# Lzcstan/DrugLAMP

Measured on AMD Instinct MI355X. Metric: drug-protein pairs/sec training step, higher is better.
Workload: dtype bf16; 1 GPU; DrugLAMP training step (cls step, epoch 1; fwd+bwd+grad all-reduce+AdamW), BindingDB-shaped synthetic pairs (512 drug nodes/tokens, 2304 protein tokens = 256 sites, pre-extracted 384-d/640-d LLM embeddings), global batch 256 = 256 per GPU x 1; per_gpu_batch=256, global_batch=256, parallelism=dp1, step_kind=cls, epoch=1, hip_graph=False, protein_seq_len=2304, distinct_batches=8, first_touch_steps=8, padding_rows=computed once, protein_cnn_rows=distinct rows, streams=independent branches on side HIP streams

## Files before the change

### druglamp_amd/_lib.py

```python
from __future__ import annotations

import ctypes as C
import os

import torch

_HERE = os.path.dirname(os.path.abspath(__file__))
_variant = os.environ.get("DL_USE_STUDY_LIB", "")
if _variant and not _variant.endswith(".so"):
    raise RuntimeError("DL_USE_STUDY_LIB=%s: the -DDL_STUDY build (libdruglamp_hip_study.so) was removed; commit 97fb613 is the last "
                       "that builds it (python -m druglamp_amd.build --study).  Only a variant library name (libdruglamp_hip_<variant>.so) "
                       "is accepted." % _variant)
LIB_PATH = os.path.join(_HERE, "lib", _variant or "libdruglamp_hip.so")

DL_F32, DL_BF16 = 0, 1

c_i64, c_i32, c_f32, c_u64, c_vp, c_sz = C.c_int64, C.c_int32, C.c_float, C.c_uint64, C.c_void_p, C.c_size_t


class ReduceItem(C.Structure):
    _fields_ = [
        ("kind", c_i32), ("out_dtype", c_i32),
        ("src", c_vp), ("out", c_vp),
        ("mn", c_i64), ("ldc", c_i64),
        ("N", c_i32), ("splits", c_i32), ("accumulate", c_i32), ("M", c_i32),
        ("cs_slabs", c_vp), ("cs_out", c_vp),
    ]


REDUCE_BATCH_MAX = 24
GEMM_GROUP_MAX = 16


class GemmArgs(C.Structure):
    _fields_ = [
        ("X", c_vp), ("ldx", c_i64), ("x_kslow", c_i32),
        ("W", c_vp), ("ldw", c_i64), ("w_kslow", c_i32),
        ("C", c_vp), ("ldc", c_i64),
        ("M", c_i64), ("N", c_i64), ("K", c_i64),
        ("in_dtype", c_i32), ("out_dtype", c_i32),
        ("bias", c_vp),
        ("residual", c_vp), ("ldr", c_i64),
        ("res_row_mod", c_i64),
        ("res_before_dropout", c_i32),
        ("act", c_i32),
        ("pre_out", c_vp), ("ldp", c_i64),
        ("dact_pre", c_vp), ("lddp", c_i64),
        ("dropout_p", c_f32), ("dropout_seed", c_u64),
        ("accumulate", c_i32),
        ("split_k", c_i32), ("workspace", c_vp), ("workspace_bytes", c_sz),
        ("x_colsum", c_vp),
        ("dropout_seed_offset", c_vp),
        ("algo", c_i32),
        ("tile_tickets", c_vp),
        ("deferred", C.POINTER(ReduceItem)),
        ("prof_tag", c_i32),
    ]


FLAG_PROT_PERIOD, FLAG_DRUG_TOKEN_PAD, FLAG_GCN_NODE_PAD, FLAG_PLAN_ROWS, FLAG_PAIR_INDEX = 1, 2, 4, 8, 16
FLAG_KEY_TABLE = 32
FLAG_MAP_COLS = 64
TAG_OTHER, TAG_QKV_OUT, TAG_FFN, TAG_CONV, TAG_WGRAD, TAG_ADAPTOR = 0, 1, 2, 3, 4, 5
TAG_NAMES = {0: "other", 1: "qkv_out", 2: "ffn", 3: "conv", 4: "wgrad", 5: "adaptor"}


class AttnFwdArgs(C.Structure):
    _fields_ = [
        ("Q", c_vp), ("K", c_vp), ("V", c_vp), ("O", c_vp), ("LSE", c_vp), ("raw_logits", c_vp),
        ("q_ps", c_i64), ("q_hs", c_i64), ("q_rs", c_i64),
        ("k_ps", c_i64), ("k_hs", c_i64), ("k_rs", c_i64),
        ("v_ps", c_i64), ("v_hs", c_i64), ("v_rs", c_i64),
        ("o_ps", c_i64), ("o_hs", c_i64), ("o_rs", c_i64), ("o_ss", c_i64),
        ("n_problems", c_i32), ("n_heads", c_i32), ("n_segments", c_i32), ("partner_shift", c_i32),
        ("Lq", c_i32), ("Lk", c_i32), ("head_dim", c_i32), ("dtype", c_i32),
        ("scale", c_f32),
        ("algo", c_i32),
        ("key_tail_rows", c_i32), ("key_tail_weight", c_f32),
    ]


class AttnBwdArgs(C.Structure):
    _fields_ = [
        ("Q", c_vp), ("K", c_vp), ("V", c_vp), ("O", c_vp), ("dO", c_vp),
        ("LSE", c_vp), ("Delta", c_vp),
        ("dQ", c_vp), ("dK", c_vp), ("dV", c_vp),
        ("q_ps", c_i64), ("q_hs", c_i64), ("q_rs", c_i64),
        ("k_ps", c_i64), ("k_hs", c_i64), ("k_rs", c_i64),
        ("v_ps", c_i64), ("v_hs", c_i64), ("v_rs", c_i64),
        ("o_ps", c_i64), ("o_hs", c_i64), ("o_rs", c_i64), ("o_ss", c_i64),
        ("do_ps", c_i64), ("do_hs", c_i64), ("do_rs", c_i64), ("do_ss", c_i64),
        ("dq_ps", c_i64), ("dq_hs", c_i64), ("dq_rs", c_i64),
        ("dk_ps", c_i64), ("dk_hs", c_i64), ("dk_rs", c_i64),
        ("dv_ps", c_i64), ("dv_hs", c_i64), ("dv_rs", c_i64),
        ("n_problems", c_i32), ("n_heads", c_i32), ("n_segments", c_i32), ("partner_shift", c_i32),
        ("Lq", c_i32), ("Lk", c_i32), ("head_dim", c_i32), ("dtype", c_i32),
        ("scale", c_f32),
        ("algo", c_i32),
        ("key_tail_rows", c_i32), ("key_tail_weight", c_f32),
    ]


class AttnProbsArgs(C.Structure):
    _fields_ = [
        ("Q", c_vp), ("K", c_vp), ("LSE", c_vp), ("out", c_vp), ("out_ld", c_i64),
        ("q_ps", c_i64), ("q_hs", c_i64), ("q_rs", c_i64),
        ("k_ps", c_i64), ("k_hs", c_i64), ("k_rs", c_i64),
        ("n_problems", c_i32), ("n_heads", c_i32), ("n_segments", c_i32), ("partner_shift", c_i32),
        ("Lq", c_i32), ("Lk", c_i32), ("head_dim", c_i32), ("dtype", c_i32),
        ("scale", c_f32),
        ("head_mean", c_i32), ("key_tail_rows", c_i32), ("key_tail_weight", c_f32), ("expand_tail", c_i32),
        ("workspace", c_vp), ("workspace_bytes", c_sz),
# ... 43 lines not shown
        ("Q", c_vp), ("K", c_vp), ("out", c_vp),
        ("q_index", c_vp), ("kv_index", c_vp), ("kv_row0", c_vp), ("kv_keys", c_vp), ("kv_tail_weight", c_vp), ("flags", c_vp),
        ("q_es", c_i64), ("q_rs", c_i64), ("k_rs", c_i64), ("out_ps", c_i64), ("out_rs", c_i64), ("kv_total_rows", c_i64),
        ("n_pairs", c_i32), ("n_q", c_i32), ("n_kv", c_i32), ("Lq", c_i32), ("head_dim", c_i32), ("dtype", c_i32),
        ("out_cols", c_i32), ("expand_tail", c_i32),
        ("scale", c_f32),
        ("key_tail_rows", c_i32),
    ]


class PgcaPairsProfileArgs(C.Structure):
    _fields_ = [
        ("Q", c_vp), ("K", c_vp), ("key_mass", c_vp), ("site_peak", c_vp), ("site_key", c_vp),
        ("q_index", c_vp), ("kv_index", c_vp), ("flags", c_vp),
        ("q_es", c_i64), ("q_rs", c_i64), ("k_es", c_i64), ("k_rs", c_i64), ("mass_ps", c_i64), ("site_ps", c_i64),
        ("n_pairs", c_i32), ("n_q", c_i32), ("n_kv", c_i32), ("Lq", c_i32), ("Lk", c_i32), ("head_dim", c_i32), ("dtype", c_i32),
        ("out_cols", c_i32),
        ("scale", c_f32),
        ("key_tail_rows", c_i32), ("key_tail_weight", c_f32),
        ("reserved", c_i32),
    ]


class PgcaPairsRaggedProfileArgs(C.Structure):
    _fields_ = [
        ("Q", c_vp), ("K", c_vp), ("key_mass", c_vp), ("site_peak", c_vp), ("site_key", c_vp),
        ("q_index", c_vp), ("kv_index", c_vp), ("kv_row0", c_vp), ("kv_keys", c_vp), ("kv_tail_weight", c_vp), ("flags", c_vp),
        ("q_es", c_i64), ("q_rs", c_i64), ("k_rs", c_i64), ("mass_ps", c_i64), ("site_ps", c_i64), ("kv_total_rows", c_i64),
        ("n_pairs", c_i32), ("n_q", c_i32), ("n_kv", c_i32), ("Lq", c_i32), ("head_dim", c_i32), ("dtype", c_i32),
        ("out_cols", c_i32),
        ("scale", c_f32),
        ("key_tail_rows", c_i32),
        ("reserved", c_i32),
    ]


class NtxentSide(C.Structure):
    _fields_ = [("q", c_vp), ("k", c_vp), ("n", c_i64), ("gid_offset", c_i64), ("lse", c_vp)]


class NtxentArgs(C.Structure):
    _fields_ = [("a", NtxentSide), ("b", NtxentSide), ("n_global", c_i64), ("d", c_i64), ("dtype", c_i32),
                ("temperature", c_f32)]


SIGNATURES = {
    "dl_last_error": (C.c_char_p, []),
    "dl_version": (c_i32, []),
    "dl_gemm_workspace_bytes": (c_sz, [C.POINTER(GemmArgs)]),
    "dl_gemm": (c_i32, [C.POINTER(GemmArgs), c_vp]),
    "dl_gemm_pair": (c_i32, [C.POINTER(GemmArgs), C.POINTER(GemmArgs), c_vp]),
    "dl_gemm_group_plan": (c_i32, [C.POINTER(GemmArgs), c_i32, C.POINTER(c_i32)]),
    "dl_gemm_group": (c_i32, [C.POINTER(GemmArgs), c_i32, c_vp]),
    "dl_reduce_batch": (c_i32, [C.POINTER(ReduceItem), c_i32, c_vp]),
    "dl_colsum": (c_i32, [c_vp, c_i64, c_i64, c_i64, c_i32, c_vp, c_i32, c_vp, c_sz, c_vp]),
    "dl_colsum_workspace_bytes": (c_sz, [c_i64, c_i64]),
    "dl_bn_workspace_bytes": (c_sz, [c_i64, c_i64]),
    "dl_bn_stats": (c_i32, [c_vp, c_i64, c_i64, c_i64, c_i64, c_i64, c_i32, c_vp, c_vp, c_sz, c_vp]),
    "dl_bn_apply_fwd": (c_i32, [c_vp, c_vp, c_vp, c_vp, c_vp, c_vp, c_i64, c_i64, c_i64, c_i64, c_i64, c_i32, c_vp]),
    "dl_bn_bwd_reduce": (c_i32, [c_vp, c_vp, c_vp, c_vp, c_i64, c_i64, c_i64, c_i64, c_i64, c_i32, c_vp, c_vp, c_sz, c_vp]),
    "dl_bn_tail_fix": (c_i32, [c_vp, c_vp, c_vp, c_vp, c_vp, c_vp, c_f32, c_i32, c_i64, c_i64, c_i64, c_i64, c_i32, c_vp]),
    "dl_bn_apply_relu_fwd": (c_i32, [c_vp, c_vp, c_vp, c_vp, c_vp, c_vp, c_i64, c_i64, c_i32, c_vp]),
    "dl_bn_relu_bwd": (c_i32, [c_vp, c_vp, c_vp, c_vp, c_vp, c_vp, c_f32, c_vp, c_vp, c_i64, c_i64, c_i32, c_vp, c_sz, c_vp]),
    "dl_bn_bwd_apply": (c_i32, [c_vp, c_vp, c_vp, c_vp, c_vp, c_vp, c_f32, c_i32, c_vp, c_i64, c_i64, c_i64, c_i64, c_i64,
                                c_i32, c_vp]),
    "dl_layernorm_fwd": (c_i32, [c_vp, c_i64, c_vp, c_vp, c_vp, c_i64, c_vp, c_vp, c_i64, c_i64, c_f32, c_i32, c_vp]),
    "dl_layernorm_bwd_workspace_bytes": (c_sz, [c_i64, c_i64]),
    "dl_layernorm_bwd": (c_i32, [c_vp, c_i64, c_i64, c_vp, c_i64, c_vp, c_vp, c_vp, c_vp, c_i64, c_vp, c_i64, c_vp, c_vp,
                                 c_i32, c_i64, c_i64, c_i32, c_vp, c_sz, C.POINTER(ReduceItem), c_vp]),
    "dl_attn_fwd": (c_i32, [C.POINTER(AttnFwdArgs), c_vp]),
    "dl_attn_bwd": (c_i32, [C.POINTER(AttnBwdArgs), c_vp]),
    "dl_attn_probs_workspace_bytes": (c_sz, [C.POINTER(AttnProbsArgs)]),
    "dl_attn_probs": (c_i32, [C.POINTER(AttnProbsArgs), c_vp]),
    "dl_pgca_pairs_fwd": (c_i32, [C.POINTER(PgcaPairsArgs), c_vp]),
    "dl_pgca_pairs_ragged_fwd": (c_i32, [C.POINTER(PgcaPairsRaggedArgs), c_vp]),
    "dl_pgca_pairs_probs": (c_i32, [C.POINTER(PgcaPairsProbsArgs), c_vp]),
    "dl_pgca_pairs_ragged_probs": (c_i32, [C.POINTER(PgcaPairsRaggedProbsArgs), c_vp]),
    "dl_pgca_pairs_profile": (c_i32, [C.POINTER(PgcaPairsProfileArgs), c_vp]),
    "dl_pgca_pairs_ragged_profile": (c_i32, [C.POINTER(PgcaPairsRaggedProfileArgs), c_vp]),
    "dl_token_gate_fwd": (c_i32, [c_vp, c_vp, c_vp, c_vp, c_i64, c_i64, c_i64, c_i32, c_i32, c_i32, c_vp]),
    "dl_token_gate_bwd": (c_i32, [c_vp, c_vp, c_vp, c_vp, c_vp, c_i64, c_i64, c_i64, c_i32, c_i32, c_i32, c_vp]),
    "dl_gate_dpre": (c_i32, [c_vp, c_vp, c_vp, c_vp, c_i64, c_i64, c_i32, c_i32, c_vp]),
    "dl_add_rowmod_dropout": (c_i32, [c_vp, c_vp, c_vp, c_i64, c_i64, c_i64, c_f32, c_u64, c_vp, c_i32, c_vp]),
    "dl_dropout_apply": (c_i32, [c_vp, c_vp, c_i64, c_i64, c_i64, c_i64, c_f32, c_u64, c_vp, c_i32, c_vp]),
    "dl_fill_pool": (c_i32, [c_vp, c_vp, c_vp, c_i64, c_i64, c_i64, c_i32, c_i32, c_i32, c_vp]),
    "dl_cnn_sitepool_fwd": (c_i32, [c_vp, c_vp, c_i64, c_i64, c_i64, c_i32, c_i32, c_i32, c_vp]),
    "dl_cnn_sitepool_bwd": (c_i32, [c_vp, c_vp, c_i64, c_i64, c_i64, c_i32, c_i32, c_i32, c_vp]),
    "dl_bn_stats_finalize": (c_i32, [c_vp, c_i64, c_i64, c_i64, c_i64, c_i64, c_vp, c_i32, c_i64, c_f32, c_f32, c_vp, c_vp, c_vp, c_vp, c_vp, c_vp, c_vp, c_sz, c_vp]),
    "dl_bn_finalize": (c_i32, [c_vp, c_i64, c_f32, c_f32, c_vp, c_vp, c_vp, c_vp, c_vp, c_i64, c_vp]),
    "dl_interleave_streams": (c_i32, [c_vp, c_vp, c_i64, c_i64, c_i32, c_i32, c_vp]),
    "dl_norm_adjacency": (c_i32, [c_vp, c_vp, c_i64, c_i32, c_i32, c_vp]),
    "dl_graph_aggregate": (c_i32, [c_vp, c_vp, c_vp, c_i64, c_i32, c_i32, c_i32, c_i32, c_i32, c_vp]),
    "dl_concat2": (c_i32, [c_vp, c_vp, c_vp, c_i64, c_i64, c_i64, c_i32, c_vp]),
    "dl_gather_pad": (c_i32, [c_vp, c_vp, c_vp, c_vp, c_i64, c_i64, c_i64, c_i32, c_i32, c_vp]),
    "dl_embed_pad": (c_i32, [c_vp, c_vp, c_vp, c_vp, c_i64, c_i64, c_i32, c_i32, c_i32, c_i32, c_vp]),
    "dl_weight_prep": (c_i32, [c_vp, c_vp, c_i32, c_i32, c_vp]),
    "dl_gelu_bwd": (c_i32, [c_vp, c_vp, c_vp, c_i64, c_i32, c_vp]),
    "dl_cast": (c_i32, [c_vp, c_i32, c_vp, c_i32, c_i64, c_vp]),
    "dl_rowmod_sum": (c_i32, [c_vp, c_vp, c_i64, c_i64, c_i64, c_i32, c_i32, c_vp]),
    "dl_cos_rowloss_fwd": (c_i32, [c_vp, c_vp, c_vp, c_vp, c_i64, c_i64, c_vp]),
    "dl_cos_rowloss_bwd": (c_i32, [c_vp, c_vp, c_f32, c_vp, c_i64, c_i64, c_vp]),
    "dl_ntxent_fwd_ex": (c_i32, [C.POINTER(NtxentArgs), c_vp, c_vp, c_vp, c_vp]),
    "dl_ntxent_bwd_ex": (c_i32, [C.POINTER(NtxentArgs), c_f32, c_vp, c_vp, c_vp]),
    "dl_ntxent_workspace_bytes": (c_sz, [c_i64, c_i64]),
    "dl_ntxent_fwd": (c_i32, [c_vp, c_vp, c_i64, c_i64, c_f32, c_vp, c_vp, c_vp, c_sz, c_vp]),
    "dl_ntxent_bwd": (c_i32, [c_vp, c_vp, c_i64, c_i64, c_f32, c_vp, c_f32, c_vp, c_vp, c_vp]),
# ... 118 lines not shown
```

### druglamp_amd/functional.py

```python
from __future__ import annotations

import functools
import contextlib
import os
import math
import weakref
from typing import List, Optional, Sequence

import torch

from . import ops

_param_epoch = 0
def _maybe_deferring():
    return contextlib.nullcontext() if os.environ.get("DL_DEFER_REDUCTIONS", "1") == "0" else ops.deferred_reductions()


def _deferring(fn):
    if os.environ.get("DL_DEFER_REDUCTIONS", "1") == "0":
        return fn

    @functools.wraps(fn)
    def wrapped(*a, **k):
        with ops.deferred_reductions():
# ... 519 lines not shown
    if not xp.is_contiguous():
        return ops.cast(x.contiguous(), dtype)
    inv = [0] * len(perm)
    for i, d in enumerate(perm):
        inv[d] = i
    return ops.cast(xp, dtype).permute(inv)


class CastFn(torch.autograd.Function):
    @staticmethod
    def forward(ctx, x, dtype):
        ctx.src = x.dtype
        return _cast_keep_layout(x, dtype)

    @staticmethod
    def backward(ctx, dy):
        return _cast_keep_layout(dy, ctx.src), None


def cast(x: torch.Tensor, dtype: torch.dtype) -> torch.Tensor:
    return x if x.dtype == dtype else CastFn.apply(x, dtype)


@torch.no_grad()
def attention_maps(x, blk, H: int, paired: bool):
    S, B, L, d = x.shape
    hd = d // H
    M = B * L
    maps = []
    qkvs = []
    for s in range(S):
        ps = blk.stream_params(s)
        xn, _, _ = ops.layernorm_fwd(x[s].reshape(M, d).contiguous(), ps[0].detach(), ps[1].detach(), 1e-6)
        w = lowp((ps[2], ps[4], ps[6]), x.dtype)
        b = lowp((ps[3], ps[5], ps[7]), torch.float32)
        qkvs.append(ops.gemm(xn, w, M=M, N=3 * d, K=d, bias=b))
    qs = (L * 3 * d, hd, 3 * d)

    def raw_of(qbuf, kbuf):
        raw = torch.empty((B, H, L, L), dtype=torch.float32, device=x.device)
        scratch = torch.empty((M, d), dtype=x.dtype, device=x.device)
        ops.attn_fwd(qbuf, kbuf[:, d:], kbuf[:, 2 * d:], n_problems=B, n_heads=H, n_segments=1, partner_shift=0, Lq=L,
                     Lk=L, head_dim=hd, scale=1.0 / math.sqrt(hd), q_strides=qs, k_strides=qs, v_strides=qs,
                     out=scratch, o_strides=(L * d, hd, d), o_ss=0, need_lse=False, raw_logits=raw)
        return torch.softmax(raw, dim=-1)

    w = raw_of(qkvs[0], qkvs[0])
    gw = raw_of(qkvs[1], qkvs[0]) if paired else None
    return w, gw


def _wgrad(g, x, M, N, K, ldx, ldw, want_bias=True, out_w=None, out_b=None):
    db = (out_b if out_b is not None else torch.empty(M, dtype=torch.float32, device=g.device)) if want_bias else None
    dw = ops.gemm(g, x, M=M, N=N, K=K, x_kslow=True, w_kslow=True, ldx=ldx, ldw=ldw, out_dtype=torch.float32,
                  split_k=0, x_colsum=db, out=out_w)
    return dw, db


class CosRowLossFn(torch.autograd.Function):

    @staticmethod
    def forward(ctx, x, y):
        x = x.float().contiguous()
        y = y.detach().float().contiguous()
        rows = ops.cos_rowloss_fwd(x, y)
        ctx.save_for_backward(x, y)
        return rows

    @staticmethod
    def backward(ctx, drows):
        x, y = ctx.saved_tensors
        dx = ops.cos_rowloss_bwd(x, y, 1.0)
        return dx * drows.unsqueeze(-1), None


class CrossEntropyRowsFn(torch.autograd.Function):

    @staticmethod
    def forward(ctx, logits, labels, C, ignore_index):
        logits = logits if logits.stride(-1) == 1 else logits.contiguous()
        labels = labels.reshape(-1).contiguous()
        out2, lse = ops.ce_rows_fwd(logits, labels, C, ignore_index)
        ctx.save_for_backward(logits, labels, lse, out2)
        ctx.cfg = (C, ignore_index)
        return out2[0]

    @staticmethod
    def backward(ctx, g):
        logits, labels, lse, out2 = ctx.saved_tensors
        C, ignore_index = ctx.cfg
        return ops.ce_rows_bwd(logits, labels, C, ignore_index, lse, out2, g.float().contiguous()), None, None, None


class NTXentFn(torch.autograd.Function):

    @staticmethod
    def forward(ctx, q, k, temperature, global_batch=False):
        import torch.distributed as dist
        if q.dtype not in (torch.float32, torch.bfloat16):
            q = q.float()
        q = q.contiguous()
        k = k.to(q.dtype).contiguous()
        world = dist.get_world_size() if (global_batch and dist.is_available() and dist.is_initialized()) else 1
        n = q.shape[0]
        if world > 1:
            rank = dist.get_rank()
# ... 267 lines not shown
        ctx.cfg = (x.shape, x.dtype)
        return x.mean(dim=1, dtype=torch.float32)

    @staticmethod
    def backward(ctx, g):
        (B, L, C), dt = ctx.cfg
        return (g * (1.0 / L)).to(dt).unsqueeze(1).expand(B, L, C)


class GraphAggregateFn(torch.autograd.Function):

    @staticmethod
    def _check(ahat, feat):
        if not (feat.is_cuda and feat.shape[-1] == 128 and ahat.dtype == feat.dtype and feat.dtype in (torch.float32, torch.bfloat16)):
            raise RuntimeError("GraphAggregateFn: device tensors of width 128 in one of fp32 / bf16 expected (got %s %s, %s %s): "
                               "there is no torch fallback" % (tuple(ahat.shape), ahat.dtype, tuple(feat.shape), feat.dtype))

    @staticmethod
    def forward(ctx, ahat, feat):
        GraphAggregateFn._check(ahat, feat)
        ctx.save_for_backward(ahat)
        return ops.graph_aggregate(ahat, feat, transpose=False)

    @staticmethod
    def backward(ctx, dout):
        (ahat,) = ctx.saved_tensors
        return None, ops.graph_aggregate(ahat, dout.contiguous(), transpose=True)


class EmbeddingFn(torch.autograd.Function):

    @staticmethod
    def forward(ctx, ids, weight, padding_idx):
        ctx.save_for_backward(ids)
        ctx.wshape = tuple(weight.shape)
        ctx.padding_idx = padding_idx
        return weight.detach()[ids]

    @staticmethod
    def backward(ctx, dy):
        (ids,) = ctx.saved_tensors
        V, D = ctx.wshape
        Vp, Dp = (V + 7) // 8 * 8, (D + 7) // 8 * 8
        flat = ids.reshape(-1)
        M = flat.numel()
        cdt = dy.dtype if dy.dtype in (torch.bfloat16, torch.float32) else torch.float32
        onehot = torch.zeros((M, Vp), dtype=cdt, device=dy.device)
        onehot.scatter_(1, flat.unsqueeze(1), 1.0)
        g = dy.reshape(M, D)
        if Dp != D or g.dtype != cdt or not g.is_contiguous():
            gp = torch.zeros((M, Dp), dtype=cdt, device=dy.device)
            gp[:, :D] = g
            g = gp
        dw = ops.gemm(onehot, g, M=Vp, N=Dp, K=M, x_kslow=True, w_kslow=True, ldx=Vp, ldw=Dp, out_dtype=torch.float32,
                      split_k=0)
        dw = dw[:V, :D]
        if ctx.padding_idx is not None:
            dw[ctx.padding_idx].zero_()
        return None, dw, None



class EmbedPadFn(torch.autograd.Function):

    @staticmethod
    def forward(ctx, ids, weight, fill, padding_idx):
        ctx.save_for_backward(ids)
        ctx.wshape = tuple(weight.shape)
        ctx.padding_idx = padding_idx
        return ops.embed_pad(ids, weight.detach(), fill, _CNN_HALO)

    @staticmethod
    def backward(ctx, dy):
        (ids,) = ctx.saved_tensors
        V, D = ctx.wshape
        B, LP, C = dy.shape
        Vp = (V + 7) // 8 * 8
        R = B * LP
        cdt = dy.dtype
        onehot = torch.zeros((B, LP, Vp), dtype=cdt, device=dy.device)
        onehot[:, _CNN_HALO:LP - _CNN_HALO].scatter_(2, ids.unsqueeze(-1), 1.0)
        g = dy.contiguous().reshape(R, C)
        dw = ops.gemm(onehot.reshape(R, Vp), g, M=Vp, N=C, K=R, x_kslow=True, w_kslow=True, ldx=Vp, ldw=C,
                      out_dtype=torch.float32, split_k=0)
        dw = dw[:V, :D]
        if ctx.padding_idx is not None:
            dw[ctx.padding_idx].zero_()
        return None, dw, None, None


class EmbedRowsFn(torch.autograd.Function):

    @staticmethod
    def forward(ctx, ids, weight, fill, padding_idx, src, period):
        ctx.save_for_backward(ids, src)
        ctx.wshape = tuple(weight.shape)
        ctx.padding_idx = padding_idx
        return ops.embed_rows(ids, weight.detach(), fill, src, period)

    @staticmethod
    def backward(ctx, dy):
        ids, src = ctx.saved_tensors
        V, D = ctx.wshape
        R, C = dy.shape
        Vp = (V + 7) // 8 * 8
        cdt = dy.dtype
        srcl = src.long()
        tok = ids.reshape(-1)[srcl.clamp(min=0)]
        onehot = torch.zeros((R, Vp), dtype=cdt, device=dy.device)
        onehot.scatter_(1, tok.unsqueeze(1), (srcl >= 0).to(cdt).unsqueeze(1))
        g = dy.contiguous()
        dw = ops.gemm(onehot, g, M=Vp, N=C, K=R, x_kslow=True, w_kslow=True, ldx=Vp, ldw=C, out_dtype=torch.float32, split_k=0)
        dw = dw[:V, :D]
        if ctx.padding_idx is not None:
            dw[ctx.padding_idx].zero_()
        return None, dw, None, None, None, None


class ExpandRowsFn(torch.autograd.Function):

    @staticmethod
    def forward(ctx, z, row_of, rep):
        ctx.save_for_backward(rep)
        return ops.rows_gather(z, row_of)

    @staticmethod
    def backward(ctx, dout):
        (rep,) = ctx.saved_tensors
        return ops.rows_sum_strided(dout.contiguous(), rep), None, None


class SitePoolRowsFn(torch.autograd.Function):

    @staticmethod
    def forward(ctx, z, row_of, rep, B, L, site_len):
        ctx.save_for_backward(row_of, rep)
        ctx.cfg = (L, site_len)
        return ops.cnn_sitepool_rows_fwd(z, row_of, B, L, site_len)

    @staticmethod
    def backward(ctx, dout):
        row_of, rep = ctx.saved_tensors
        L, site_len = ctx.cfg
        return ops.cnn_sitepool_rows_bwd(dout, rep, row_of, L, site_len), None, None, None, None, None


class SitePoolFn(torch.autograd.Function):

    @staticmethod
    def forward(ctx, z, site_len):
        B, L, C = z.shape
        ctx.cfg = (L, site_len)
        return ops.cnn_sitepool_fwd(z.contiguous(), L, 0, site_len)

    @staticmethod
    def backward(ctx, dout):
        L, site_len = ctx.cfg
        return ops.cnn_sitepool_bwd(dout, L, 0, site_len), None


class FillPoolFn(torch.autograd.Function):

    @staticmethod
    def forward(ctx, x, site_len, out_dtype):
        ctx.cfg = (tuple(x.shape), x.dtype, int(site_len))
# ... 198 lines not shown
```

### druglamp_amd/ops.py

```python
from __future__ import annotations

import contextlib
import ctypes as C
import math
import os
from typing import Optional

import torch

from . import _lib
from ._lib import (DL_BF16, DL_F32, AttnBwdArgs, AttnFwdArgs, AttnProbsArgs, GemmArgs, PgcaPairsArgs, PgcaPairsProbsArgs, PgcaPairsProfileArgs,
                   PgcaPairsRaggedArgs, PgcaPairsRaggedProbsArgs, PgcaPairsRaggedProfileArgs, check)

_DT = {torch.float32: DL_F32, torch.bfloat16: DL_BF16}


def _dt(t: torch.Tensor) -> int:
    try:
        return _DT[t.dtype]
    except KeyError:
        raise TypeError("druglamp_amd: unsupported dtype %s (float32 / bfloat16 only)" % t.dtype)


_raw_stream = getattr(torch._C, "_cuda_getCurrentRawStream", None)
# ... 77 lines not shown
    a.bias = _ptr(bias)
    a.residual = _ptr(residual)
    a.ldr = N if residual is None else residual.stride(-2)
    a.res_row_mod = res_row_mod
    a.res_before_dropout = int(res_before_dropout)
    a.act = act
    a.pre_out = _ptr(pre_out)
    a.ldp = N
    a.dact_pre = _ptr(dact_pre)
    a.lddp = N
    a.dropout_p = float(dropout_p)
    a.dropout_seed = int(seed)
    a.accumulate = int(accumulate)
    a.split_k = split_k
    a.x_colsum = _ptr(x_colsum)
    a.dropout_seed_offset = _seed_offset_ptr(x.device) if dropout_p > 0 else None
    a.algo = algo
    a.tile_tickets = _tickets_ptr(x.device)
    a.prof_tag = _lib.TAG_WGRAD if (x_kslow and w_kslow and _prof_tag != _lib.TAG_CONV) else _prof_tag
    return a, out


def gemm(x: torch.Tensor, w: torch.Tensor, **kw) -> torch.Tensor:
    a, out = _gemm_args(x, w, **kw)
    accumulate, x_colsum = kw.get("accumulate", False), kw.get("x_colsum")
    if (_wgroup is not None and a.x_kslow and a.w_kslow and a.split_k == 0 and not accumulate
            and (a.K <= group_wgrad_max_k or a.M * a.N < group_wgrad_small_mn)
            and x.dtype == torch.bfloat16 and out.dtype == torch.float32 and a.bias is None and a.residual is None and not a.act):
        _wgroup.append((a, out, x_colsum, x, w))
        return out
    _gemm_launch(a, out, x, accumulate, x_colsum)
    return out


def _gemm_launch(a, out, x, accumulate, x_colsum) -> None:
    L = _lib.lib()
    if accumulate and (_pending or _wgroup):
        flush_reductions()
    nbytes = L.dl_gemm_workspace_bytes(C.byref(a))
    item = None
    if nbytes:
        if _pending is not None and not accumulate:
            ws = torch.empty(nbytes, dtype=torch.uint8, device=x.device)
            item = _lib.ReduceItem()
            a.deferred = C.pointer(item)
        else:
            ws = _ws.get(nbytes, x.device)
        a.workspace, a.workspace_bytes = ws.data_ptr(), ws.numel()
    check(L.dl_gemm(C.byref(a), _stream()), "dl_gemm")
    if item is not None and item.kind != 0:
        _pending.append((item, ws, out, x_colsum))


group_wgrad_max_k = int(os.environ.get("DL_GROUP_WGRAD_MAX_K", "65536"))
group_wgrad_small_mn = int(os.environ.get("DL_GROUP_WGRAD_SMALL_MN", "655360"))
group_wgrad_min_n = 2
_wgroup = None


def flush_wgrads() -> None:
    if not _wgroup:
        return
    L = _lib.lib()
    todo = list(_wgroup)
    del _wgroup[:]
    for i in range(0, len(todo), _lib.GEMM_GROUP_MAX):
        part = todo[i:i + _lib.GEMM_GROUP_MAX]
        n = len(part)
        arr = (GemmArgs * n)(*[t[0] for t in part])
        splits = (C.c_int32 * n)()
        if n < group_wgrad_min_n or L.dl_gemm_group_plan(arr, n, splits) != 0:
            for a, out, x_colsum, x, _w in part:
                _gemm_launch(a, out, x, False, x_colsum)
            continue
        keep = []
        for k, (a, out, x_colsum, x, _w) in enumerate(part):
            nbytes = int(splits[k]) * a.M * (a.N + (1 if x_colsum is not None else 0)) * 4
            ws = torch.empty(nbytes, dtype=torch.uint8, device=x.device)
            item = _lib.ReduceItem()
            arr[k].workspace, arr[k].workspace_bytes = ws.data_ptr(), nbytes
            arr[k].deferred = C.pointer(item)
            keep.append((item, ws, out, x_colsum))
        check(L.dl_gemm_group(arr, n, _stream()), "dl_gemm_group")
        _pending.extend(keep)


def gemm_pair(xs, ws, **kw):
    L = _lib.lib()
    per = [{k: (v[i] if isinstance(v, (tuple, list)) else v) for k, v in kw.items()} for i in range(2)]
    (a0, o0), (a1, o1) = _gemm_args(xs[0], ws[0], **per[0]), _gemm_args(xs[1], ws[1], **per[1])
    if L.dl_gemm_workspace_bytes(C.byref(a0)) or L.dl_gemm_workspace_bytes(C.byref(a1)):
        return gemm(xs[0], ws[0], **per[0]), gemm(xs[1], ws[1], **per[1])
    check(L.dl_gemm_pair(C.byref(a0), C.byref(a1), _stream()), "dl_gemm_pair")
    return o0, o1


_pending = None


@contextlib.contextmanager
def deferred_reductions():
    global _pending, _wgroup
    if _pending is not None:
        yield
        return
    _pending = []
# ... 962 lines not shown
```

### include/druglamp_hip.h

```cpp
#ifndef DRUGLAMP_HIP_H
#define DRUGLAMP_HIP_H

#include <stddef.h>
#include <stdint.h>

#ifdef __cplusplus
extern "C" {
#endif

typedef enum { DL_OK = 0, DL_ERR_ARG = -1, DL_ERR_SHAPE = -2, DL_ERR_ALIGN = -3,
               DL_ERR_WORKSPACE = -4, DL_ERR_LAUNCH = -5, DL_ERR_UNSUPPORTED = -6 } dl_status;

typedef enum { DL_F32 = 0, DL_BF16 = 1 } dl_dtype;

typedef void* dl_stream;

const char* dl_last_error(void);
int dl_version(void);

typedef struct dl_reduce_item {
  int32_t kind;
  int32_t out_dtype;
  const float* src;
  void* out;
  int64_t mn;
  int64_t ldc;
  int32_t N;
  int32_t splits;
  int32_t accumulate;
  int32_t M;
  const float* cs_slabs;
  float* cs_out;
} dl_reduce_item;
enum { DL_REDUCE_NONE = 0, DL_REDUCE_SPLITK = 1, DL_REDUCE_PARTIALS = 2 };
enum { DL_REDUCE_BATCH_MAX = 24 };
int dl_reduce_batch(const dl_reduce_item* items, int32_t n, dl_stream s);

typedef struct {
  const void* X; int64_t ldx; int32_t x_kslow;
  const void* W; int64_t ldw; int32_t w_kslow;
  void* C; int64_t ldc;
  int64_t M, N, K;
  int32_t in_dtype, out_dtype;
  const float* bias;
  const void* residual; int64_t ldr;
  int64_t res_row_mod;
  int32_t res_before_dropout;
  int32_t act;
  void* pre_out; int64_t ldp;
  const void* dact_pre; int64_t lddp;
  float dropout_p; uint64_t dropout_seed;
  int32_t accumulate;
  int32_t split_k; void* workspace; size_t workspace_bytes;
  float* x_colsum;
  const uint64_t* dropout_seed_offset;
  int32_t algo;
  int32_t* tile_tickets;
  dl_reduce_item* deferred;
  int32_t prof_tag;
} dl_gemm_args;
enum { DL_TAG_OTHER = 0, DL_TAG_QKV_OUT = 1, DL_TAG_FFN = 2, DL_TAG_CONV = 3, DL_TAG_WGRAD = 4, DL_TAG_ADAPTOR = 5 };
enum { DL_GEMM_ALGO_AUTO = 0, DL_GEMM_ALGO_TILE128 = 1 };

size_t dl_gemm_workspace_bytes(const dl_gemm_args* a);
int dl_gemm(const dl_gemm_args* a, dl_stream s);
int dl_gemm_pair(const dl_gemm_args* a, const dl_gemm_args* b, dl_stream s);
int dl_gemm_group_plan(const dl_gemm_args* args, int32_t n, int32_t* splits_out);
int dl_gemm_group(const dl_gemm_args* args, int32_t n, dl_stream s);

int dl_colsum(const void* X, int64_t ldx, int64_t M, int64_t N, int32_t dtype, float* out,
              int32_t accumulate, void* workspace, size_t workspace_bytes, dl_stream s);
size_t dl_colsum_workspace_bytes(int64_t M, int64_t N);

size_t dl_bn_workspace_bytes(int64_t R, int64_t C);
int dl_bn_stats(const void* y, int64_t R, int64_t C, int64_t win, int64_t halo, int64_t valid,
                int32_t dtype, float* sums, void* workspace, size_t workspace_bytes, dl_stream s);
int dl_bn_finalize(const float* sums, int64_t n, float eps, float momentum, float* mean, float* var, float* rstd,
                   float* running_mean, float* running_var, int64_t C, dl_stream s);
int dl_bn_apply_fwd(const void* y, void* z, const float* mean, const float* rstd, const float* gamma,
                    const float* beta, int64_t R, int64_t C, int64_t win, int64_t halo, int64_t valid,
                    int32_t dtype, dl_stream s);
int dl_bn_bwd_reduce(const void* dz, const void* y, const float* mean, const float* rstd, int64_t R,
                     int64_t C, int64_t win, int64_t halo, int64_t valid, int32_t dtype, float* sums,
                     void* workspace, size_t workspace_bytes, dl_stream s);
int dl_bn_bwd_apply(const void* dz, const void* y, const float* mean, const float* rstd,
                    const float* gamma, const float* sums, float inv_n, int32_t relu_mask, void* dy,
                    int64_t R, int64_t C, int64_t win, int64_t halo, int64_t valid, int32_t dtype,
                    dl_stream s);
int dl_bn_stats_rw(const void* y, int64_t R, int64_t C, const float* row_w, int32_t dtype, float* sums, void* workspace,
                   size_t workspace_bytes, dl_stream s);
int dl_bn_stats_finalize(const void* y, int64_t R, int64_t C, int64_t win, int64_t halo, int64_t valid, const float* row_w,
                         int32_t dtype, int64_t n, float eps, float momentum, float* sums, float* mean, float* var, float* rstd,
                         float* running_mean, float* running_var, void* workspace, size_t workspace_bytes, dl_stream s);
int dl_bn_apply_fwd_rw(const void* y, void* z, const float* mean, const float* rstd, const float* gamma, const float* beta,
                       int64_t R, int64_t C, const float* row_w, int32_t dtype, dl_stream s);
int dl_bn_bwd_reduce_rw(const void* dz, const void* y, const float* mean, const float* rstd, int64_t R, int64_t C,
                        const float* row_w, int32_t dtype, float* sums, void* workspace, size_t workspace_bytes, dl_stream s);
int dl_bn_bwd_apply_rw(const void* dz, const void* y, const float* mean, const float* rstd, const float* gamma,
                       const float* sums, float inv_n, int32_t relu_mask, void* dy, int64_t R, int64_t C, const float* row_w,
                       int32_t dtype, dl_stream s);
int dl_bn_tail_fix(void* dy, const void* y, const float* mean, const float* rstd, const float* gamma, const float* sums,
                   float inv_n, int32_t w, int64_t R, int64_t C, int64_t win, int64_t lead, int32_t dtype, dl_stream s);
int dl_bn_apply_relu_fwd(const void* y, void* z, const float* mean, const float* rstd, const float* gamma, const float* beta,
                         int64_t R, int64_t C, int32_t dtype, dl_stream s);
int dl_bn_relu_bwd(const void* dz, const void* y, const float* mean, const float* rstd, const float* gamma, const float* beta,
                   float inv_n, void* dy, float* sums, int64_t R, int64_t C, int32_t dtype, void* workspace, size_t workspace_bytes,
                   dl_stream s);
int dl_bn_eval_bwd(const void* dz, const void* y, const float* mean, const float* rstd, const float* gamma, const float* beta,
                   int32_t relu_in, int32_t relu_out, void* dy, float* sums, int64_t R, int64_t C, int64_t win, int64_t halo,
                   int64_t valid, const float* row_w, int32_t dtype, void* workspace, size_t workspace_bytes, dl_stream s);

int dl_layernorm_fwd(const void* x, int64_t ldx, const float* gamma, const float* beta, void* y,
                     int64_t ldy, float* mean, float* rstd, int64_t M, int64_t D, float eps,
                     int32_t dtype, dl_stream s);
size_t dl_layernorm_bwd_workspace_bytes(int64_t M, int64_t D);
int dl_layernorm_bwd(const void* dy, int64_t lddy, int64_t dy_share, const void* x, int64_t ldx, const float* mean,
                     const float* rstd, const float* gamma, const void* dres, int64_t lddres,
                     void* dx, int64_t lddx, float* dgamma, float* dbeta, int32_t accumulate,
                     int64_t M, int64_t D, int32_t dtype, void* workspace, size_t workspace_bytes,
                     dl_reduce_item* deferred, dl_stream s);

// ... 228 lines not shown
```

Before: 21870 pairs/s.

## Add split-K weight-gradient kernel for small-output, long-K GEMMs

```diff
diff --git a/druglamp_amd/_lib.py b/druglamp_amd/_lib.py
--- a/druglamp_amd/_lib.py
+++ b/druglamp_amd/_lib.py
@@ -58,6 +58,28 @@
     ]
 
 
+class WgradSmallArgs(C.Structure):
+    _fields_ = [
+        ("X", c_vp), ("ldx", c_i64),
+        ("W", c_vp), ("ldw", c_i64),
+        ("C", c_vp), ("ldc", c_i64),
+        ("M", c_i64), ("N", c_i64), ("K", c_i64),
+        ("in_dtype", c_i32), ("out_dtype", c_i32),
+        ("x_kslow", c_i32), ("w_kslow", c_i32),
+        ("accumulate", c_i32),
+        ("with_colsum", c_i32),
+        ("x_colsum", c_vp),
+        ("tile", c_i32), ("splits", c_i32),
+        ("workspace", c_vp), ("workspace_bytes", c_sz),
+        ("prof_tag", c_i32),
+    ]
+
+
+class WgradSmallPlan(C.Structure):
+    _fields_ = [("eligible", c_i32), ("preferred", c_i32), ("tile", c_i32), ("splits", c_i32), ("k_per_split", c_i64),
+                ("workspace_bytes", c_sz)]
+
+
 FLAG_PROT_PERIOD, FLAG_DRUG_TOKEN_PAD, FLAG_GCN_NODE_PAD, FLAG_PLAN_ROWS, FLAG_PAIR_INDEX = 1, 2, 4, 8, 16
 FLAG_KEY_TABLE = 32
 FLAG_MAP_COLS = 64
@@ -207,6 +229,9 @@
     "dl_gemm_pair": (c_i32, [C.POINTER(GemmArgs), C.POINTER(GemmArgs), c_vp]),
     "dl_gemm_group_plan": (c_i32, [C.POINTER(GemmArgs), c_i32, C.POINTER(c_i32)]),
     "dl_gemm_group": (c_i32, [C.POINTER(GemmArgs), c_i32, c_vp]),
+    "dl_wgrad_small_plan_query": (c_i32, [C.POINTER(WgradSmallArgs), C.POINTER(WgradSmallPlan)]),
+    "dl_wgrad_small_workspace_bytes": (c_sz, [C.POINTER(WgradSmallArgs)]),
+    "dl_wgrad_small": (c_i32, [C.POINTER(WgradSmallArgs), c_vp]),
     "dl_reduce_batch": (c_i32, [C.POINTER(ReduceItem), c_i32, c_vp]),
     "dl_colsum": (c_i32, [c_vp, c_i64, c_i64, c_i64, c_i32, c_vp, c_i32, c_vp, c_sz, c_vp]),
     "dl_colsum_workspace_bytes": (c_sz, [c_i64, c_i64]),
diff --git a/druglamp_amd/csrc/wgrad_small.hip b/druglamp_amd/csrc/wgrad_small.hip
--- /dev/null
+++ b/druglamp_amd/csrc/wgrad_small.hip
@@ -0,0 +1,312 @@
+#include <stdint.h>
+#include <algorithm>
+#include <type_traits>
+#include "common.cuh"
+
+namespace {
+
+constexpr int NTHREADS = 256;
+constexpr int KSTEP = 64;
+constexpr int MIN_STEPS = 8;
+constexpr int SLAB_FRACTION = 2;
+constexpr int64_t MAX_MN = 655360;
+constexpr int64_t PREFER_MIN_K = 2048;
+constexpr double PREFER_MAX_WORK = 1.0e10;
+constexpr int RED_THREADS = 1024;
+constexpr int RED_POS = 16, RED_ZL = RED_THREADS / RED_POS;
+
+struct WsP {
+  const char* X; const char* W;
+  int64_t ldx, ldw;
+  int M, N, K, k_per_split, mt, nt, splits;
+  float* slabs;
+  float* cs_slabs;
+};
+
+template <int TW> __device__ __forceinline__ constexpr int swz(int k) {
+  if constexpr (TW == 4) return ((k & 3) << 1) | (((k >> 3) & 1) << 3);
+  else return (((k >> 1) & 1) << 1) | (((k >> 3) & 1) << 2);
+}
+
+template <int TW>
+__device__ __forceinline__ void load_tile(const char* base, int64_t ld, int c0, int ncols, int k0, int kend, u32x4 (&r)[TW]) {
+  constexpr int CPR = 4 * TW;
+#pragma unroll
+  for (int i = 0; i < TW; ++i) {
+    const int c = threadIdx.x + i * NTHREADS;
+    const int krow = c / CPR, cc = c % CPR;
+    const int gk = k0 + krow, gc = c0 + cc * 8;
+    u32x4 v = {0u, 0u, 0u, 0u};
+    if (gk < kend && gc < ncols) v = *reinterpret_cast<const u32x4*>(base + ((int64_t)gk * ld + gc) * 2);
+    r[i] = v;
+  }
+}
+template <int TW>
+__device__ __forceinline__ void store_tile(char* lds, const u32x4 (&r)[TW]) {
+  constexpr int CPR = 4 * TW, PITCH = 64 * TW;
+#pragma unroll
+  for (int i = 0; i < TW; ++i) {
+    const int c = threadIdx.x + i * NTHREADS;
+    const int krow = c / CPR, cc = c % CPR;
+    lds_write16(lds, krow * PITCH + ((cc ^ swz<TW>(krow)) << 4), r[i]);
+  }
+}
+template <int TW>
+__device__ __forceinline__ u32x4 read_frag(const char* lds, int rb, int kf, int il, int g) {
+  constexpr int PITCH = 64 * TW;
+  const int kidx = kf * 32 + g * 8 + (il >> 2);
+  const int cb = (rb + (il & 3) * 4) * 2;
+  const u32x2 a = lds_read_tr16(lds, kidx * PITCH + (((cb >> 4) ^ swz<TW>(kidx)) << 4) + (cb & 15));
+  const u32x2 b = lds_read_tr16(lds, (kidx + 4) * PITCH + (((cb >> 4) ^ swz<TW>(kidx + 4)) << 4) + (cb & 15));
+  u32x4 r = {a[0], a[1], b[0], b[1]};
+  return r;
+}
+
+template <int TW, bool CS>
+__global__ __launch_bounds__(NTHREADS) void wgrad_small_kernel(const WsP p) {
+  constexpr int BT = 32 * TW, TB = KSTEP * BT * 2;
+  __shared__ __attribute__((aligned(16))) char smem[4 * TB];
+  const int tid = threadIdx.x, lane = tid & 63, wave = tid >> 6;
+  const int il = lane & 15, g = lane >> 4;
+  const int wm = wave >> 1, wn = wave & 1;
+
+  const uint32_t t = xcd_remap(blockIdx.x, gridDim.x);
+  const int tiles = p.mt * p.nt;
+  const int split = (int)(t / (uint32_t)tiles), tile = (int)(t % (uint32_t)tiles);
+  const int m0 = (tile / p.nt) * BT, n0 = (tile % p.nt) * BT;
+  const int kbeg = split * p.k_per_split;
+  const int kend = min(p.K, kbeg + p.k_per_split);
+  const int nk = (kend - kbeg + KSTEP - 1) / KSTEP;
+
+  f32x4 acc[TW][TW];
+#pragma unroll
+  for (int i = 0; i < TW; ++i)
+#pragma unroll
+    for (int j = 0; j < TW; ++j) acc[i][j] = f32x4{0.f, 0.f, 0.f, 0.f};
+  float cs[TW];
+#pragma unroll
+  for (int i = 0; i < TW; ++i) cs[i] = 0.f;
+  const bool do_cs = CS && n0 == 0 && wn == 0;
+
+  constexpr int DEPTH = TW == 2 ? 4 : 2;
+  u32x4 rx[DEPTH][TW], rw[DEPTH][TW];
+#pragma unroll
+  for (int d = 0; d < DEPTH; ++d) {
+    load_tile<TW>(p.X, p.ldx, m0, p.M, kbeg + d * KSTEP, kend, rx[d]);
+    load_tile<TW>(p.W, p.ldw, n0, p.N, kbeg + d * KSTEP, kend, rw[d]);
+  }
+
+  auto step = [&](u32x4 (&rx)[TW], u32x4 (&rw)[TW], int kt, auto with_cs) {
+    constexpr bool WCS = decltype(with_cs)::value;
+    char* buf = smem + (kt & 1) * 2 * TB;
+    store_tile<TW>(buf, rx);
+    store_tile<TW>(buf + TB, rw);
+    const int kn = kbeg + (kt + DEPTH) * KSTEP;
+    load_tile<TW>(p.X, p.ldx, m0, p.M, kn, kend, rx);
+    load_tile<TW>(p.W, p.ldw, n0, p.N, kn, kend, rw);
+    __syncthreads();
+#pragma unroll
+    for (int kf = 0; kf < KSTEP / 32; ++kf) {
+      u32x4 fx[TW], fw[TW];
+#pragma unroll
+      for (int i = 0; i < TW; ++i) fx[i] = read_frag<TW>(buf, wm * 16 * TW + i * 16, kf, il, g);
+#pragma unroll
+      for (int j = 0; j < TW; ++j) fw[j] = read_frag<TW>(buf + TB, wn * 16 * TW + j * 16, kf, il, g);
+#pragma unroll
+      for (int i = 0; i < TW; ++i)
+#pragma unroll
+        for (int j = 0; j < TW; ++j) acc[i][j] = Mma<bf16_t>::mma(fw[j], fx[i], acc[i][j]);
+      if constexpr (WCS) {
+#pragma unroll
+        for (int i = 0; i < TW; ++i) cs[i] = frag_slot_sum<bf16_t>(fx[i], cs[i]);
+      }
+    }
+  };
+  auto kloop = [&](auto with_cs) {
+    for (int kt = 0; kt < nk; kt += DEPTH) {
+#pragma unroll
+      for (int d = 0; d < DEPTH; ++d)
+        if (kt + d < nk) step(rx[d], rw[d], kt + d, with_cs);
+    }
+  };
+  if constexpr (CS) {
+    if (do_cs) kloop(std::true_type{}); else kloop(std::false_type{});
+  } else {
+    kloop(std::false_type{});
+  }
+
+  if constexpr (CS) {
+    if (do_cs) {
+#pragma unroll
+      for (int i = 0; i < TW; ++i) {
+        const float v = group4_sum(cs[i]);
+        const int m = m0 + wm * 16 * TW + i * 16 + il;
+        if (g == 0 && m < p.M) p.cs_slabs[(int64_t)split * p.M + m] = v;
+      }
+    }
+  }
+#pragma unroll
+  for (int i = 0; i < TW; ++i) {
+    const int m = m0 + wm * 16 * TW + i * 16 + il;
+#pragma unroll
+    for (int j = 0; j < TW; ++j) {
+      const int n = n0 + wn * 16 * TW + j * 16 + 4 * g;
+      if (m < p.M && n < p.N)
+        *reinterpret_cast<f32x4*>(p.slabs + ((int64_t)split * p.M + m) * p.N + n) = acc[i][j];
+    }
+  }
+}
+
+template <typename V>
+__device__ __forceinline__ V slab_sum(const float* __restrict__ first, int64_t stride, int splits, bool live, char* lds) {
+  V* red = reinterpret_cast<V*>(lds);
+  V* red2 = red + RED_ZL * RED_POS;
+  const int pos = threadIdx.x % RED_POS, zl = threadIdx.x / RED_POS;
+  V s = V(0.f);
+  if (live) {
+    for (int z0 = zl; z0 < splits; z0 += 4 * RED_ZL) {
+      V v[4];
+#pragma unroll
+      for (int k = 0; k < 4; ++k) {
+        const int z = z0 + k * RED_ZL;
+        v[k] = z < splits ? *reinterpret_cast<const V*>(first + (int64_t)z * stride) : V(0.f);
+      }
+      s += v[0]; s += v[1]; s += v[2]; s += v[3];
+    }
+  }
+  red[zl * RED_POS + pos] = s;
+  __syncthreads();
+  if (zl < 8) {
+    V t = red[(zl * 8) * RED_POS + pos];
+#pragma unroll
+    for (int j = 1; j < 8; ++j) t += red[(zl * 8 + j) * RED_POS + pos];
+    red2[zl * RED_POS + pos] = t;
+  }
+  __syncthreads();
+  V t = red2[pos];
+#pragma unroll
+  for (int j = 1; j < 8; ++j) t += red2[j * RED_POS + pos];
+  return t;
+}
+
+__global__ __launch_bounds__(RED_THREADS) void wgrad_small_reduce_kernel(const float* __restrict__ slabs, float* __restrict__ out,
+                                                                         int64_t mn, int64_t ldc, int N, int splits, int accumulate,
+                                                                         const float* __restrict__ cs_slabs, float* __restrict__ cs_out,
+                                                                         int M, uint32_t main_blocks) {
+  __shared__ __attribute__((aligned(16))) char lds[(RED_ZL + 8) * RED_POS * sizeof(f32x4)];
+  const int pos = threadIdx.x % RED_POS, zl = threadIdx.x / RED_POS;
+  if (blockIdx.x >= main_blocks) {
+    const int m = (int)(blockIdx.x - main_blocks) * RED_POS + pos;
+    const bool live = m < M;
+    const float t = slab_sum<float>(cs_slabs + (live ? m : 0), M, splits, live, lds);
+    if (live && zl == 0) cs_out[m] = t;
+    return;
+  }
+  const int64_t i4 = ((int64_t)blockIdx.x * RED_POS + pos) * 4;
+  const bool live = i4 < mn;
+  f32x4 t = slab_sum<f32x4>(slabs + (live ? i4 : 0), mn, splits, live, lds);
+  if (!live || zl != 0) return;
+  const int64_t m = i4 / N, n = i4 % N;
+  float* dst = out + m * ldc + n;
+  if (accumulate) t += *reinterpret_cast<const f32x4*>(dst);
+  *reinterpret_cast<f32x4*>(dst) = t;
+}
+
+bool supported(const dl_wgrad_small_args* a) {
+  if (!a) return false;
+  if (a->in_dtype != DL_BF16 || a->out_dtype != DL_F32 || !a->x_kslow || !a->w_kslow) return false;
+  if (a->M < 8 || a->N < 8 || a->K < 1 || a->M % 8 != 0 || a->N % 8 != 0) return false;
+  if (a->M * a->N > MAX_MN || a->K >= (1ll << 30)) return false;
+  if (a->ldx < a->M || a->ldw < a->N || a->ldc < a->N || a->ldx % 8 != 0 || a->ldw % 8 != 0 || a->ldc % 4 != 0) return false;
+  if ((((uintptr_t)a->X | (uintptr_t)a->W | (uintptr_t)a->C | (uintptr_t)a->x_colsum) & 15) != 0) return false;
+  if (a->tile != 0 && a->tile != 64 && a->tile != 128) return false;
+  return true;
+}
+
+void make_plan(const dl_wgrad_small_args* a, dl_wgrad_small_plan* pl) {
+  *pl = dl_wgrad_small_plan{};
+  if (!supported(a)) return;
+  const int64_t M = a->M, N = a->N, K = a->K;
+  const int64_t ksteps = (K + KSTEP - 1) / KSTEP;
+  auto slabs_for = [&](int bt, int64_t* per_out) {
+    const int64_t tiles = ((M + bt - 1) / bt) * ((N + bt - 1) / bt);
+    const int64_t resident = 256 * (bt == 64 ? 4 : 2);
+    int64_t sp = a->splits > 0 ? a->splits : std::min(std::min(resident / tiles, ksteps / MIN_STEPS),
+                                                      K * (M + N) * 2 / SLAB_FRACTION / (M * N * 4));
+    sp = std::max<int64_t>(1, std::min(sp, ksteps));
+    const int64_t per = (ksteps + sp - 1) / sp;
+    *per_out = per;
+    return (ksteps + per - 1) / per;
+  };
+  int64_t per = 0, sp = 0;
+  int bt = a->tile;
+  if (bt == 0) {
+    bt = 64;
+    if (M > 64 && N > 64 && M * N > 128 * 256) {
+      sp = slabs_for(128, &per);
+      if (((M + 127) / 128) * ((N + 127) / 128) * sp >= 256) bt = 128;
+    }
+  }
+  sp = slabs_for(bt, &per);
+  pl->eligible = 1;
+  pl->preferred = (K >= PREFER_MIN_K && (double)M * (double)N * (double)K < PREFER_MAX_WORK) ? 1 : 0;
+  pl->tile = bt;
+  pl->splits = (int32_t)sp;
+  pl->k_per_split = per * KSTEP;
+  pl->workspace_bytes = (size_t)sp * (size_t)M * (size_t)(N + ((a->with_colsum || a->x_colsum) ? 1 : 0)) * sizeof(float);
+}
+
+}
+
+extern "C" int dl_wgrad_small_plan_query(const dl_wgrad_small_args* a, dl_wgrad_small_plan* plan) {
+  DL_CHECK_ARG(a && plan, DL_ERR_ARG, "dl_wgrad_small_plan_query: null argument");
+  make_plan(a, plan);
+  return DL_OK;
+}
+
+extern "C" size_t dl_wgrad_small_workspace_bytes(const dl_wgrad_small_args* a) {
+  if (!a) return 0;
+  dl_wgrad_small_plan pl;
+  make_plan(a, &pl);
+  return pl.eligible ? pl.workspace_bytes : 0;
+}
+
+extern "C" int dl_wgrad_small(const dl_wgrad_small_args* a, dl_stream stream) {
+  hipStream_t s = (hipStream_t)stream;
+  DL_CHECK_ARG(a && a->X && a->W && a->C, DL_ERR_ARG, "dl_wgrad_small: null operand");
+  dl_wgrad_small_plan pl;
+  make_plan(a, &pl);
+  DL_CHECK_ARG(pl.eligible, DL_ERR_UNSUPPORTED,
+               "dl_wgrad_small: not eligible (bf16 K-slow operands, f32 output, M, N multiples of 8, M * N <= %ld, pitches multiples "
+               "of 8 (ldc: 4), 16-byte aligned pointers); use dl_gemm", (long)MAX_MN);
+  DL_CHECK_ARG(a->workspace && a->workspace_bytes >= pl.workspace_bytes && ((uintptr_t)a->workspace & 15) == 0, DL_ERR_WORKSPACE,
+               "dl_wgrad_small: needs %zu workspace bytes (16-byte aligned), got %zu", pl.workspace_bytes, a->workspace_bytes);
+  WsP p;
+  p.X = (const char*)a->X; p.W = (const char*)a->W; p.ldx = a->ldx; p.ldw = a->ldw;
+  p.M = (int)a->M; p.N = (int)a->N; p.K = (int)a->K;
+  p.k_per_split = (int)pl.k_per_split; p.splits = pl.splits;
+  p.mt = (int)((a->M + pl.tile - 1) / pl.tile); p.nt = (int)((a->N + pl.tile - 1) / pl.tile);
+  p.slabs = (float*)a->workspace;
+  p.cs_slabs = a->x_colsum ? p.slabs + (size_t)pl.splits * a->M * a->N : nullptr;
+  const uint32_t nblocks = (uint32_t)p.mt * p.nt * p.splits;
+  dl_prof_before(0, s);
+  if (pl.tile == 64) {
+    if (p.cs_slabs) hipLaunchKernelGGL((wgrad_small_kernel<2, true>), dim3(nblocks), dim3(NTHREADS), 0, s, p);
+    else hipLaunchKernelGGL((wgrad_small_kernel<2, false>), dim3(nblocks), dim3(NTHREADS), 0, s, p);
+  } else {
+    if (p.cs_slabs) hipLaunchKernelGGL((wgrad_small_kernel<4, true>), dim3(nblocks), dim3(NTHREADS), 0, s, p);
+    else hipLaunchKernelGGL((wgrad_small_kernel<4, false>), dim3(nblocks), dim3(NTHREADS), 0, s, p);
+  }
+  DL_CHECK_LAUNCH("dl_wgrad_small");
+  const double mn_d = (double)a->M * (double)a->N;
+  dl_prof_after(0, s, 2.0 * mn_d * (double)a->K,
+                (double)a->K * (double)(a->M + a->N) * 2.0 + mn_d * 4.0 * (a->accumulate ? 2.0 : 1.0), a->prof_tag);
+  const int64_t mn = a->M * a->N;
+  const int64_t blocks = (mn / 4 + RED_POS - 1) / RED_POS;
+  const int64_t cs_blocks = a->x_colsum ? (a->M + RED_POS - 1) / RED_POS : 0;
+  hipLaunchKernelGGL(wgrad_small_reduce_kernel, dim3((uint32_t)(blocks + cs_blocks)), dim3(RED_THREADS), 0, s,
+                     (const float*)p.slabs, a->C, mn, a->ldc, (int)a->N, (int)pl.splits, a->accumulate,
+                     (const float*)p.cs_slabs, a->x_colsum, (int)a->M, (uint32_t)blocks);
+  DL_CHECK_LAUNCH("dl_wgrad_small(reduce)");
+  return DL_OK;
+}
diff --git a/druglamp_amd/functional.py b/druglamp_amd/functional.py
--- a/druglamp_amd/functional.py
+++ b/druglamp_amd/functional.py
@@ -595,6 +595,8 @@
 
 def _wgrad(g, x, M, N, K, ldx, ldw, want_bias=True, out_w=None, out_b=None):
     db = (out_b if out_b is not None else torch.empty(M, dtype=torch.float32, device=g.device)) if want_bias else None
+    if ops.wgrad_small_takes(g, x, M=M, N=N, K=K, ldx=ldx, ldw=ldw, out=out_w, x_colsum=db):
+        return ops.wgrad_small(g, x, M=M, N=N, K=K, ldx=ldx, ldw=ldw, out=out_w, x_colsum=db), db
     dw = ops.gemm(g, x, M=M, N=N, K=K, x_kslow=True, w_kslow=True, ldx=ldx, ldw=ldw, out_dtype=torch.float32,
                   split_k=0, x_colsum=db, out=out_w)
     return dw, db
@@ -968,8 +970,7 @@
             gp = torch.zeros((M, Dp), dtype=cdt, device=dy.device)
             gp[:, :D] = g
             g = gp
-        dw = ops.gemm(onehot, g, M=Vp, N=Dp, K=M, x_kslow=True, w_kslow=True, ldx=Vp, ldw=Dp, out_dtype=torch.float32,
-                      split_k=0)
+        dw, _ = _wgrad(onehot, g, Vp, Dp, M, Vp, Dp, want_bias=False)
         dw = dw[:V, :D]
         if ctx.padding_idx is not None:
             dw[ctx.padding_idx].zero_()
@@ -997,8 +998,7 @@
         onehot = torch.zeros((B, LP, Vp), dtype=cdt, device=dy.device)
         onehot[:, _CNN_HALO:LP - _CNN_HALO].scatter_(2, ids.unsqueeze(-1), 1.0)
         g = dy.contiguous().reshape(R, C)
-        dw = ops.gemm(onehot.reshape(R, Vp), g, M=Vp, N=C, K=R, x_kslow=True, w_kslow=True, ldx=Vp, ldw=C,
-                      out_dtype=torch.float32, split_k=0)
+        dw, _ = _wgrad(onehot.reshape(R, Vp), g, Vp, C, R, Vp, C, want_bias=False)
         dw = dw[:V, :D]
         if ctx.padding_idx is not None:
             dw[ctx.padding_idx].zero_()
@@ -1026,7 +1026,7 @@
         onehot = torch.zeros((R, Vp), dtype=cdt, device=dy.device)
         onehot.scatter_(1, tok.unsqueeze(1), (srcl >= 0).to(cdt).unsqueeze(1))
         g = dy.contiguous()
-        dw = ops.gemm(onehot, g, M=Vp, N=C, K=R, x_kslow=True, w_kslow=True, ldx=Vp, ldw=C, out_dtype=torch.float32, split_k=0)
+        dw, _ = _wgrad(onehot, g, Vp, C, R, Vp, C, want_bias=False)
         dw = dw[:V, :D]
         if ctx.padding_idx is not None:
             dw[ctx.padding_idx].zero_()
diff --git a/druglamp_amd/ops.py b/druglamp_amd/ops.py
--- a/druglamp_amd/ops.py
+++ b/druglamp_amd/ops.py
@@ -153,6 +153,59 @@
         _pending.append((item, ws, out, x_colsum))
 
 
+WGRAD_SMALL = os.environ.get("DL_WGRAD_SMALL", "1") != "0"
+
+
+def _wgrad_small_args(x, w, out, M, N, K, ldx, ldw, accumulate, x_colsum, tile=0, splits=0):
+    a = _lib.WgradSmallArgs()
+    a.X, a.W, a.C = x.data_ptr(), w.data_ptr(), _ptr(out)
+    a.ldx, a.ldw = ldx, ldw
+    a.ldc = N if out is None else (out.stride(0) if out.dim() == 2 else N)
+    a.M, a.N, a.K = M, N, K
+    a.in_dtype = _DT.get(x.dtype, -1) if x.dtype == w.dtype else -1
+    a.out_dtype = DL_F32 if out is None else _DT.get(out.dtype, -1)
+    a.x_kslow = a.w_kslow = 1
+    a.accumulate = int(accumulate)
+    a.x_colsum = _ptr(x_colsum)
+    a.tile, a.splits = tile, splits
+    a.prof_tag = _lib.TAG_WGRAD if _prof_tag != _lib.TAG_CONV else _prof_tag
+    return a
+
+
+def wgrad_small_plan(x, w, *, M, N, K, ldx=None, ldw=None, out=None, accumulate=False, x_colsum=None, tile=0, splits=0):
+    a = _wgrad_small_args(x, w, out, M, N, K, ldx or M, ldw or N, accumulate, x_colsum, tile, splits)
+    plan = _lib.WgradSmallPlan()
+    check(_lib.lib().dl_wgrad_small_plan_query(C.byref(a), C.byref(plan)), "dl_wgrad_small_plan_query")
+    return plan
+
+
+def wgrad_small_takes(x, w, *, M, N, K, ldx, ldw, out=None, x_colsum=None) -> bool:
+    if not WGRAD_SMALL or x.dtype != torch.bfloat16 or w.dtype != torch.bfloat16 or (out is not None and out.dtype != torch.float32):
+        return False
+    if _wgroup is not None and (K <= group_wgrad_max_k or M * N < group_wgrad_small_mn):
+        return False
+    plan = wgrad_small_plan(x, w, M=M, N=N, K=K, ldx=ldx, ldw=ldw, out=out, x_colsum=x_colsum)
+    return bool(plan.eligible and plan.preferred)
+
+
+def wgrad_small(x: torch.Tensor, w: torch.Tensor, *, M: int, N: int, K: int, ldx: Optional[int] = None, ldw: Optional[int] = None,
+                out=None, accumulate=False, x_colsum=None, tile=0, splits=0) -> torch.Tensor:
+    _need_gpu(x, w)
+    if out is None:
+        if accumulate:
+            raise ValueError("wgrad_small: accumulate needs `out`")
+        out = torch.empty((M, N), dtype=torch.float32, device=x.device)
+    a = _wgrad_small_args(x, w, out, M, N, K, ldx or M, ldw or N, accumulate, x_colsum, tile, splits)
+    L = _lib.lib()
+    if accumulate and (_pending or _wgroup):
+        flush_reductions()
+    nbytes = L.dl_wgrad_small_workspace_bytes(C.byref(a))
+    ws = _ws.get(nbytes, x.device)
+    a.workspace, a.workspace_bytes = ws.data_ptr(), ws.numel()
+    check(L.dl_wgrad_small(C.byref(a), _stream()), "dl_wgrad_small")
+    return out
+
+
 group_wgrad_max_k = int(os.environ.get("DL_GROUP_WGRAD_MAX_K", "65536"))
 group_wgrad_small_mn = int(os.environ.get("DL_GROUP_WGRAD_SMALL_MN", "655360"))
 group_wgrad_min_n = 2
diff --git a/include/druglamp_hip.h b/include/druglamp_hip.h
--- a/include/druglamp_hip.h
+++ b/include/druglamp_hip.h
@@ -67,6 +67,31 @@
 int dl_gemm_pair(const dl_gemm_args* a, const dl_gemm_args* b, dl_stream s);
 int dl_gemm_group_plan(const dl_gemm_args* args, int32_t n, int32_t* splits_out);
 int dl_gemm_group(const dl_gemm_args* args, int32_t n, dl_stream s);
+
+typedef struct {
+  const void* X; int64_t ldx;
+  const void* W; int64_t ldw;
+  float* C; int64_t ldc;
+  int64_t M, N, K;
+  int32_t in_dtype, out_dtype;
+  int32_t x_kslow, w_kslow;
+  int32_t accumulate;
+  int32_t with_colsum;
+  float* x_colsum;
+  int32_t tile;
+  int32_t splits;
+  void* workspace; size_t workspace_bytes;
+  int32_t prof_tag;
+} dl_wgrad_small_args;
+typedef struct {
+  int32_t eligible, preferred;
+  int32_t tile, splits;
+  int64_t k_per_split;
+  size_t workspace_bytes;
+} dl_wgrad_small_plan;
+int dl_wgrad_small_plan_query(const dl_wgrad_small_args* a, dl_wgrad_small_plan* plan);
+size_t dl_wgrad_small_workspace_bytes(const dl_wgrad_small_args* a);
+int dl_wgrad_small(const dl_wgrad_small_args* a, dl_stream s);
 
 int dl_colsum(const void* X, int64_t ldx, int64_t M, int64_t N, int32_t dtype, float* out,
               int32_t accumulate, void* workspace, size_t workspace_bytes, dl_stream s);
```

Result: no change. 21920 pairs/s (median of 6 runs) (+0.2%).
